# Juzhan/TAP-Net

Hardware: AMD Instinct MI355X
Metric: env-steps/s (batch placements) 2D n=10 LB_GREEDY; 1/2/4/8 GPU + CPU ref (higher is better)
Workload: dtype i32 height-maps / f64 candidate scores / f32 masks

## Files before the change

tap-net_amd/csrc/rolling.hip:

```cpp
#include <new>

#include "tap_common.h"
#include "tap_masks.h"
#include "tap_place.h"
#include "tap_waves.h"

struct RollArgs {
    int B, D, N, child, W, L, H, arm;
    const int32_t *blocks;
    const int32_t *positions;
    unsigned long long *rel;
    unsigned long long *state;
    const int64_t *remove_ptr;
    float *static_out;
    float *dynamic_out;
    float *colsum_out;
    unsigned long long *bits_out;
    float *cur_mask_out;
    int32_t *nodes_out;
    int32_t *err_out;
    int err_sticky;
    int wt;
};

__device__ __forceinline__ LaneRole roll_lane_role(int v, const float *dy, int C4, int RP, int rows)
{
#ifdef TAP_STREAM_UNALIGNED
    const int add = 0;
#else
    const int add = ((RP * C4) & 3) == 0 ? (int)((reinterpret_cast<uintptr_t>(dy) >> 4) & 3) : 0;
#endif
    return stream_lane_role(v, 0, C4, RP, 65536 / C4 + 1, 0, add, (rows + RP - 1) / RP);
}

__device__ __forceinline__ bool rng_meet(int a0, int a1, int b0, int b1) { return a0 < b1 && b0 < a1; }

template <int D>
__global__ void __launch_bounds__(TAP_BLOCK) k_rolling_init(RollArgs a)
{
    __shared__ int s_blk[TAP_BLOCK / 64][64 * 3];
    __shared__ int s_pos[TAP_BLOCK / 64][64 * 3];
    const int w = threadIdx.x >> 6, b = threadIdx.x & 63;
    const int inst = blockIdx.x * (TAP_BLOCK / 64) + w;
    const int n = a.N;
    if (inst < a.B)
        for (int k = b; k < n * D; k += 64) {
            s_blk[w][k] = a.blocks[(size_t)inst * n * D + k];
            s_pos[w][k] = a.positions[(size_t)inst * n * D + k];
        }
    tap_wave_lds_sync();
    if (inst >= a.B) return;
    if (b == 0) { a.state[(size_t)inst * 2] = 0; a.state[(size_t)inst * 2 + 1] = 0; }
    if (b >= n) return;
    const int *blk = s_blk[w], *pos = s_pos[w];
#define BX(i) blk[(i) * D]
#define BY(i) (D == 3 ? blk[(i) * D + 1] : 1)
// ... 348 lines not shown
                    if (dy) dy[(size_t)(sec * child + rm) * nRc + col] = (float)((m[sec] >> node) & 1ull);
            }
        }
    }
    
    if (!packed) return;
    tap_wave_lds_sync();
    PROF(6);
    const int C4 = nRc >> 2, RP = 64 / C4;
    if (dy && v < RP * C4) {
        const LaneRole role = roll_lane_role(v, dy, C4, RP, rows);
        const int c4 = role.c4;
        const u64 w0 = S.cw[c4 * 4], w1 = S.cw[c4 * 4 + 1], w2 = S.cw[c4 * 4 + 2], w3 = S.cw[c4 * 4 + 3];
        float4 *dst = reinterpret_cast<float4 *>(dy) + c4;
        int rw = role.r0;
        for (int i = 0; i < role.nq; ++i, rw += RP) {
            if ((unsigned)rw >= (unsigned)rows) continue;
            store_stream(&dst[(size_t)rw * C4], make_float4(bit_as_float(w0, rw), bit_as_float(w1, rw), bit_as_float(w2, rw),
                                                            bit_as_float(w3, rw)), a.wt);
        }
    }
    PROF(7);
}

template <int D, int CH>
__device__ __forceinline__ void rolling_emit_fast_tail(const RollArgs &a, int inst, int v, RollLds &S)
{
    constexpr int R = D == 2 ? 2 : 6, NRC = CH * R, C4 = NRC / 4, RP = 64 / C4, ROWS = 3 * CH, QN = (ROWS + RP - 1) / RP;
#if defined(TAP_PROF)
    long long tp = clock64();
#endif
    float *st = a.static_out + (size_t)inst * (1 + D) * NRC;
    float *dy = a.dynamic_out ? a.dynamic_out + (size_t)inst * ROWS * NRC : nullptr;
    if (v < NRC) {
        const int col = v, r = v / CH, cm = v - r * CH;
        const int pz = D == 3 ? (0x126 >> (2 * r)) & 3 : 1 - r;
        const bool guarded = pz == 0 || (D == 3 && pz == 1);
        const int k1 = pz == 0 ? 1 : 3;
        const unsigned ws0 = S.f.iw[cm];
        const unsigned r1 = S.f.iw[k1 * CH + cm], r2 = S.f.iw[(k1 + 1) * CH + cm];
        const unsigned ws1 = guarded ? r1 : 0u, ws2 = guarded ? r2 : 0u;
        const int c0 = __popc(ws0), c1 = __popc(ws1), c2 = __popc(ws2);
        if (a.colsum_out) {
            a.colsum_out[((size_t)inst * 3 + 0) * NRC + col] = (float)c0;
            a.colsum_out[((size_t)inst * 3 + 1) * NRC + col] = (float)c1;
            a.colsum_out[((size_t)inst * 3 + 2) * NRC + col] = (float)c2;
        }
        if (a.cur_mask_out) a.cur_mask_out[(size_t)inst * NRC + col] = (c1 * c2 + c0 != 0) ? 0.f : 1.f;
        const unsigned w = ws0 | (ws1 << CH) | (ws2 << (2 * CH));
        S.f.cw32[col] = w;
        if (a.bits_out) a.bits_out[(size_t)inst * NRC + col] = (u64)w;
        st[col] = (float)cm;
        const int r4 = 4 * r;
        const int o0 = D == 3 ? (0x884400 >> r4) & 15 : (0x40 >> r4) & 15;
        const int o1 = D == 3 ? (0x408084 >> r4) & 15 : (0x04 >> r4) & 15;
        const char *row = reinterpret_cast<const char *>(&S.f.dims[cm][0]);
        st[(size_t)1 * NRC + col] = (float)*reinterpret_cast<const int *>(row + o0);
        st[(size_t)2 * NRC + col] = (float)*reinterpret_cast<const int *>(row + o1);
        if (D == 3) {
            const int o2 = (0x040848 >> r4) & 15;
            st[(size_t)3 * NRC + col] = (float)*reinterpret_cast<const int *>(row + o2);
        }
    }
    tap_wave_lds_sync();
    PROF(6);
    {
        constexpr int K = RP * C4;
        constexpr bool AL = (K & 3) == 0;
#ifdef TAP_STREAM_UNALIGNED
        const int sb = 0;
#else
        const int sb = AL ? __builtin_amdgcn_readfirstlane((int)((reinterpret_cast<uintptr_t>(dy) >> 4) & 3)) : 0;
#endif
        if (dy && v < K) {
            int role = v - sb;
            const int late = role < 0 ? 1 : 0;
            role += late ? K : 0;
            const int rsub = role / C4, c4 = role - rsub * C4;
            const uint4 cq = *reinterpret_cast<const uint4 *>(&S.f.cw32[c4 * 4]);
            unsigned mk = 0u;
#pragma unroll
            for (int q = 0; q < QN; ++q) mk |= 1u << (RP * q);
            unsigned il = (cq.x >> rsub) & mk;
            il |= ((cq.y >> rsub) & mk) << 1;
            il |= ((cq.z >> rsub) & mk) << 2;
            il |= ((cq.w >> rsub) & mk) << 3;
            float4 *dst = reinterpret_cast<float4 *>(dy) + c4 + (size_t)rsub * C4;
            constexpr int NI = QN + ((AL && RP * (QN - 1) + (K - 3) / C4 < ROWS) ? 1 : 0);
            int q = -late;
#pragma unroll
            for (int i = 0; i < NI; ++i, ++q) {
                if (q >= 0 && RP * q + rsub < ROWS) {
                    const unsigned nib = (il >> (RP * q)) & 15u;
                    store_stream(&dst[(size_t)RP * q * C4], *reinterpret_cast<const float4 *>(&S.f.lut[nib][0]), a.wt);
                }
            }
        }
// ... 700 lines not shown
                               uint64_t *bits_out, float *current_mask_out, int32_t *nodes_out,
                               int32_t *err_out, void *stream, int err_sticky);

extern "C" int tap_rolling_window(tap_ctx *ctx, int B, int D, int N, int child, const int32_t *blocks,
                                  const uint64_t *rel, uint64_t *state, const int64_t *remove_ptr,
                                  float *static_out, float *dynamic_out, float *colsum_out,
                                  uint64_t *bits_out, float *current_mask_out, int32_t *nodes_out,
                                  int32_t *err_out, void *stream)
{
    return rolling_window_impl(ctx, B, D, N, child, blocks, rel, state, remove_ptr, static_out, dynamic_out, colsum_out,
                               bits_out, current_mask_out, nodes_out, err_out, stream, 0);
}

static int rolling_window_impl(tap_ctx *ctx, int B, int D, int N, int child, const int32_t *blocks,
                               const uint64_t *rel, uint64_t *state, const int64_t *remove_ptr,
                               float *static_out, float *dynamic_out, float *colsum_out,
                               uint64_t *bits_out, float *current_mask_out, int32_t *nodes_out,
                               int32_t *err_out, void *stream, int err_sticky)
{
    int rc = roll_check(ctx, B, D, N, child);
    if (rc) return rc;
    if (!blocks || !rel || !state || !static_out) return tap_fail(ctx, TAP_E_INVALID, "null pointer");
    if (!dynamic_out && !bits_out)
        return tap_fail(ctx, TAP_E_INVALID, "dynamic_out may only be left out when bits_out takes the window's bit shadow");
    RollArgs a = {};
    a.err_sticky = err_sticky;
    a.wt = tap_write_through((size_t)B * 3 * child * child * (D == 2 ? 2 : 6) * sizeof(float));
    a.B = B; a.D = D; a.N = N; a.child = child; a.blocks = blocks;
    a.rel = reinterpret_cast<unsigned long long *>(const_cast<uint64_t *>(rel));
    a.state = reinterpret_cast<unsigned long long *>(state);
    a.remove_ptr = remove_ptr; a.static_out = static_out; a.dynamic_out = dynamic_out;
    a.colsum_out = colsum_out; a.cur_mask_out = current_mask_out; a.nodes_out = nodes_out; a.err_out = err_out;
    a.bits_out = reinterpret_cast<unsigned long long *>(bits_out);
    if (bits_out && (3 * child > 64 || (child * (D == 2 ? 2 : 6)) % 4 != 0 || child * (D == 2 ? 2 : 6) > 256))
        return tap_fail(ctx, TAP_E_UNSUPPORTED, "bits_out needs 3*child <= 64, (child*R) %% 4 == 0, child*R <= 256");
    const int grid = (B + TAP_BLOCK / 64 - 1) / (TAP_BLOCK / 64);
    if (grid == 0) return TAP_OK;
    if (const int nw = roll_wide_nw(N, child)) {
        hipStream_t s_ = (hipStream_t)stream;
#define TAP_ROLL_WIDE(D_) do { \
            if (nw == 2) hipLaunchKernelGGL((k_rolling_window<D_, ROLL_CH_WIDE>), dim3(grid), dim3(TAP_BLOCK), 0, s_, ROLL_HOT_ARGS(a), a); \
            else if (nw == 3) hipLaunchKernelGGL((k_rolling_window_wide<D_, 3>), dim3(grid), dim3(TAP_BLOCK), 0, s_, ROLL_HOT_ARGS(a), a); \
            else hipLaunchKernelGGL((k_rolling_window_wide<D_, 4>), dim3(grid), dim3(TAP_BLOCK), 0, s_, ROLL_HOT_ARGS(a), a); } while (0)
        if (D == 2) TAP_ROLL_WIDE(2); else TAP_ROLL_WIDE(3);
#undef TAP_ROLL_WIDE
        TAP_LAUNCH_CHECK(ctx, "k_rolling_window(wide)");
        tap_variant_hit(ctx, TAP_HIT_ROLL_WINDOW, D, 0, nw == 2 ? TapVariant{0, ROLL_CH_WIDE, 0} : TapVariant{1, nw, 0}, a.wt);
        return TAP_OK;
    }
    if (N > 64) {
        const int g2 = (B + 63) / 64;
        hipStream_t s_ = (hipStream_t)stream;
#define TAP_ROLL_BIG(D_) do { \
            if (N <= 256) hipLaunchKernelGGL((k_rolling_window_big<D_, 4>), dim3(g2), dim3(64), 0, s_, a); \
            else if (N <= 1024) hipLaunchKernelGGL((k_rolling_window_big<D_, 16>), dim3(g2), dim3(64), 0, s_, a); \
            else hipLaunchKernelGGL((k_rolling_window_big<D_, 64>), dim3(g2), dim3(64), 0, s_, a); } while (0)
        if (D == 2) TAP_ROLL_BIG(2); else TAP_ROLL_BIG(3);
#undef TAP_ROLL_BIG
        TAP_LAUNCH_CHECK(ctx, "k_rolling_window_big");
        tap_variant_hit(ctx, TAP_HIT_ROLL_WINDOW, D, 0, TapVariant{2, 0, N <= 256 ? 4 : N <= 1024 ? 16 : 64}, a.wt);
        return TAP_OK;
    }
    const bool fast = roll_fast_ok(D, child);
    if (D == 2) {
        if (fast) hipLaunchKernelGGL((k_rolling_window<2, 10>), dim3(grid), dim3(TAP_BLOCK), 0, (hipStream_t)stream, ROLL_HOT_ARGS(a), a);
        else hipLaunchKernelGGL((k_rolling_window<2, 0>), dim3(grid), dim3(TAP_BLOCK), 0, (hipStream_t)stream, ROLL_HOT_ARGS(a), a);
// ... 44 lines not shown
{
    int rc = tap_desc_validate(ctx, d);
    if (rc) return rc;
    if (d->B == 0) return TAP_OK;
    rc = roll_check(ctx, d->B, d->D, N, child);
    if (rc) return rc;
    if (!env_state || !blocks || !rel || !state || !ptr || !static_cur || !static_next || static_cur == static_next)
        return tap_fail(ctx, TAP_E_INVALID, "bad rolling_step arguments (static_cur and static_next must differ)");
    if (!dynamic_out && !bits_out)
        return tap_fail(ctx, TAP_E_INVALID, "dynamic_out may only be left out when bits_out takes the window's bit shadow");
    if (d->strategy != TAP_LB_GREEDY || tap_is_big(d) || (N > 64 && roll_wide_nw(N, child) != 2)) {
        rc = tap_env_step_gather(ctx, d, env_state, static_cur, 1 + d->D, child * (d->D == 2 ? 2 : 6), ptr, nullptr,
                                 feature_out, stream);
        if (rc == TAP_OK && aux) {
            StepArgs s = {};
            s.d = *d; s.static_ = static_cur; s.static_rows = 1 + d->D; s.nR = child * (d->D == 2 ? 2 : 6); s.ptr = ptr;
            s.dec_static_out = aux->dec_static_out; s.tour_out = aux->tour_out; s.picked_out = aux->picked_out;
            s.nodes_cur = aux->nodes_cur; s.child = child; s.tour_stride = aux->tour_stride; s.tour_col = aux->tour_col;
            rc = tap_step_aux_launch(ctx, s, (hipStream_t)stream);
        }
        return rc ? rc : rolling_window_impl(ctx, d->B, d->D, N, child, blocks, rel, state, ptr, static_next, dynamic_out,
                                             colsum_out, bits_out, current_mask_out, nodes_out, err_out, stream, aux != nullptr);
    }
    RollStepArgs a = {};
    const int R = d->D == 2 ? 2 : 6;
    a.r.err_sticky = aux != nullptr;
    a.r.wt = tap_write_through((size_t)d->B * 3 * child * child * R * sizeof(float));
    a.r.B = d->B; a.r.D = d->D; a.r.N = N; a.r.child = child; a.r.blocks = blocks;
    a.r.rel = reinterpret_cast<unsigned long long *>(const_cast<uint64_t *>(rel));
    a.r.state = reinterpret_cast<unsigned long long *>(state);
    a.r.remove_ptr = ptr; a.r.static_out = static_next; a.r.dynamic_out = dynamic_out;
    a.r.colsum_out = colsum_out; a.r.cur_mask_out = current_mask_out; a.r.nodes_out = nodes_out; a.r.err_out = err_out;
    a.r.bits_out = reinterpret_cast<unsigned long long *>(bits_out);
    if (bits_out && (3 * child > 64 || (child * R) % 4 != 0 || child * R > 256))
        return tap_fail(ctx, TAP_E_UNSUPPORTED, "bits_out needs 3*child <= 64, (child*R) %% 4 == 0, child*R <= 256");
    a.s.d = *d;
    tap_env_layout(d, env_state, &a.s.v);
    a.s.static_ = static_cur; a.s.static_rows = 1 + d->D; a.s.nR = child * R; a.s.ptr = ptr;
    a.s.feature_out = feature_out; a.s.flen = tap_env_feature_len(d);
    a.s.lut = ctx ? ctx->stab_lut : nullptr;
    if (aux) {
        a.s.dec_static_out = aux->dec_static_out; a.s.tour_out = aux->tour_out; a.s.picked_out = aux->picked_out;
        a.s.nodes_cur = aux->nodes_cur; a.s.child = child; a.s.tour_stride = aux->tour_stride; a.s.tour_col = aux->tour_col;
    }
    const int Gs = tap_group_size(d);
    hipStream_t st = (hipStream_t)stream;
    if (d->D == 2) {
        if (Gs == 8) return launch_rolling_step<2, 8>(ctx, a, st);
        if (Gs == 16) return launch_rolling_step<2, 16>(ctx, a, st);
        if (Gs == 32) return launch_rolling_step<2, 32>(ctx, a, st);
        return launch_rolling_step<2, 64>(ctx, a, st);
    }
    if (Gs == 8) return launch_rolling_step<3, 8>(ctx, a, st);
    if (Gs == 16) return launch_rolling_step<3, 16>(ctx, a, st);
    if (Gs == 32) return launch_rolling_step<3, 32>(ctx, a, st);
    return launch_rolling_step<3, 64>(ctx, a, st);
}

extern "C" int tap_rolling_step(tap_ctx *ctx, const tap_env_desc *d, void *env_state, int N, int child,
                                const int32_t *blocks, const uint64_t *rel, uint64_t *state,
                                const int64_t *ptr, const float *static_cur, float *static_next,
                                float *dynamic_out, float *colsum_out, uint64_t *bits_out,
                                float *current_mask_out, int32_t *nodes_out, int32_t *err_out,
                                float *feature_out, void *stream)
{
    return rolling_step_impl(ctx, d, env_state, N, child, blocks, rel, state, ptr, static_cur, static_next, dynamic_out,
// ... 93 lines not shown
```

tap-net_amd/csrc/tap_masks.h:

```cpp
#pragma once

#include <hip/hip_runtime.h>

#include <cstdint>
#include <type_traits>
#include <cstdlib>

#include "tap_stream_variant.h"

constexpr size_t TAP_WT_MAX_BYTES = 64u << 20;

struct MaskArgs {
    int B, n, R, nR, rows, update_rows, static_rows;
    const float *dyn_in;
    float *dyn_out;
    const float *static_;
    const int64_t *ptr;
    const float *mask_in;
    const float *cs_in;
    float *cs_out;
    float *cur_out;
    float *mask_out;
    const unsigned long long *bits_in;
    unsigned long long *bits_out;
    int *nonbinary;
    int c4_magic, rp;
    int wt;
    int sb_mul, sb_add, nq, nq2;
    int inplace;
};

inline int tap_write_through(size_t bytes);

constexpr int TAP_HOT_MAGIC_MASK = 0xffffff, TAP_HOT_SB_MUL_SHIFT = 24, TAP_HOT_SB_ADD_SHIFT = 26, TAP_HOT_SB_MASK = 3;

inline MaskArgs mask_finish(MaskArgs a)
{
    const int c4 = a.nR >> 2;
    a.c4_magic = c4 > 0 ? 65536 / c4 + 1 : 0;
    static_assert(65536 + 1 <= TAP_HOT_MAGIC_MASK, "c4_magic shares its kernel argument with sb_mul / sb_add (TAP_MASK_HOT_ARGS)");
    a.rp = c4 > 0 ? 64 / c4 : 0;
    a.wt = tap_write_through((size_t)a.B * a.rows * a.nR * sizeof(float));
    const bool al = a.wt && c4 > 0 && ((a.rp * c4) & 3) == 0;
    a.sb_mul = al ? (a.rows * c4) & 3 : 0;
    a.sb_add = al ? (int)((reinterpret_cast<uintptr_t>(a.dyn_out) >> 4) & 3) : 0;
    a.nq = a.rp > 0 ? (a.rows + a.rp - 1) / a.rp : 0;
    a.nq2 = a.rp > 0 ? (2 * a.rows + a.rp - 1) / a.rp : 0;
    return a;
}

struct LaneRole {
    int rsub, c4;
    int r0;
    int nq;
    int sb;
};

__device__ __forceinline__ LaneRole stream_lane_role(int lane, int env, int C4, int RP, int c4_magic, int sb_mul, int sb_add, int nq)
{
    const int sb = __builtin_amdgcn_readfirstlane((env * sb_mul + sb_add) & 3);
    int role = lane - sb;
    const bool late = role < 0;
    role += late ? RP * C4 : 0;
    LaneRole o;
    o.rsub = (int)(((unsigned)role * (unsigned)c4_magic) >> 16);
    o.c4 = role - o.rsub * C4;
    o.r0 = o.rsub - (late ? RP : 0);
    o.nq = nq + (sb != 0);
    o.sb = sb;
    return o;
}

__host__ __device__ __forceinline__ bool mask_builds_bits(const MaskArgs &a) { return !a.bits_in && a.bits_out && a.dyn_in; }

#define TAP_MASK_HOT_PARAMS const int64_t *h_ptr, const float *h_static, const float *h_mask_in, const void *h_src, int h_B, \
                            int h_nR, int h_static_rows, int h_c4_magic
#define TAP_MASK_HOT_NAMES h_ptr, h_static, h_mask_in, h_src, h_B, h_nR, h_static_rows, h_c4_magic
#define TAP_MASK_HOT_ARGS(m) (m).ptr, (m).static_, (m).mask_in,                                                              \
        ((m).bits_in ? static_cast<const void *>((m).bits_in) : static_cast<const void *>((m).dyn_in)), (m).B, (m).nR,       \
        (m).static_rows, ((m).c4_magic | (((m).sb_mul & TAP_HOT_SB_MASK) << TAP_HOT_SB_MUL_SHIFT) |                           \
                          (((m).sb_add & TAP_HOT_SB_MASK) << TAP_HOT_SB_ADD_SHIFT))
__device__ __forceinline__ MaskArgs tap_mask_hot(const MaskArgs &k, bool src_is_bits, TAP_MASK_HOT_PARAMS)
{
    MaskArgs m = k;
    m.ptr = h_ptr; m.static_ = h_static; m.mask_in = h_mask_in;
    m.B = h_B; m.nR = h_nR; m.static_rows = h_static_rows; m.c4_magic = h_c4_magic & TAP_HOT_MAGIC_MASK;
    m.sb_mul = (h_c4_magic >> TAP_HOT_SB_MUL_SHIFT) & TAP_HOT_SB_MASK; m.sb_add = (h_c4_magic >> TAP_HOT_SB_ADD_SHIFT) & TAP_HOT_SB_MASK;
    if (src_is_bits) m.bits_in = static_cast<const unsigned long long *>(h_src);
    else m.dyn_in = static_cast<const float *>(h_src);
    return m;
}


#ifdef TAP_PROF
constexpr int TAP_PROF_WGS = 2048, TAP_PROF_WAVES = 16;
static __device__ unsigned long long tap_prof_tl[TAP_PROF_WGS * TAP_PROF_WAVES * 4];
#define TL_STAMP(i) do { if ((threadIdx.x & 63) == 0 && blockIdx.x < TAP_PROF_WGS) \
        tap_prof_tl[(blockIdx.x * TAP_PROF_WAVES + (threadIdx.x >> 6)) * 4 + (i)] = __builtin_amdgcn_s_memrealtime(); } while (0)
#define TL_WAIT_VM() __builtin_amdgcn_s_waitcnt(0)
#else
#define TL_STAMP(i) do { } while (0)
#define TL_WAIT_VM() do { } while (0)
#endif

__device__ __forceinline__ void tap_wave_lds_sync_m()
{
    __builtin_amdgcn_fence(__ATOMIC_RELEASE, "wavefront");
    __builtin_amdgcn_wave_barrier();
    __builtin_amdgcn_fence(__ATOMIC_ACQUIRE, "wavefront");
}

__device__ __forceinline__ void store_stream(float4 *dst, const float4 &v, int wt)
{
    typedef float v4f __attribute__((ext_vector_type(4)));
    const v4f nv = {v.x, v.y, v.z, v.w};
    if (wt) asm volatile("global_store_dwordx4 %0, %1, off sc0 sc1\n\ts_nop 1" : : "v"(dst), "v"(nv) : "memory");
    else __builtin_nontemporal_store(nv, reinterpret_cast<v4f *>(dst));
}

inline int tap_write_through(size_t bytes, size_t limit)
{
    static const int forced = [] { const char *e = getenv("TAP_WRITE_THROUGH"); return e ? (e[0] != '0') : -1; }();
    if (forced >= 0) return forced;
    return bytes <= limit;
}
inline int tap_write_through(size_t bytes) { return tap_write_through(bytes, TAP_WT_MAX_BYTES); }

__device__ __forceinline__ float bit_as_float(unsigned long long w, int r)
{
    const unsigned half = r < 32 ? (unsigned)w : (unsigned)(w >> 32);
    return (float)((half >> (r & 31)) & 1u);
}

__device__ __forceinline__ long tap_mod_col(long p, int n, int nR)
{
    if ((unsigned long)p >= (unsigned long)nR) p = 0;
    while (p >= n) p -= n;
    return p;
}

__device__ __forceinline__ void mask_column(const MaskArgs &a, int env, int j, long real_m,
                                            float move, float small, float large)
{
    float keep = a.mask_in ? a.mask_in[(size_t)env * a.nR + j] : 1.f;
    if (a.ptr)
        for (int r = 0; r < a.R; ++r)
            if (j == real_m + (long)a.n * r) keep = 0.f;
    if (a.mask_out) a.mask_out[(size_t)env * a.nR + j] = keep;
// ... 200 lines not shown
    for (int r = 0; r < 5; ++r) v = v >= n ? v - n : v;
    while (v >= n) v -= n;
    return v;
}

template <int NS, int NC, bool BUILD = false, bool MERGED = true, int C4S = 0, bool INPLACE = false, bool FULL = false>
__device__ __forceinline__ void stream_wave_bits_r4(const MaskArgs &a, int senv0, int lane, const bool (&on_)[NS],
                                                 float *lds = nullptr)
{
    static_assert(!(BUILD && INPLACE), "the first step on a fresh tensor writes all of it");
    bool on[NS];
#pragma unroll
    for (int k = 0; k < NS; ++k) on[k] = FULL ? true : on_[k];
#if defined(TAP_STREAM_LOAD_BJ)
    constexpr bool BJ_X = false;
#elif defined(TAP_STREAM_BJX_ALL)
    constexpr bool BJ_X = !BUILD && NC == 1 && (C4S == 5 || C4S == 15);
#else
    constexpr bool BJ_X = !BUILD && NC == 1 && NS == 1 && (C4S == 5 || C4S == 15);
#endif
    typedef unsigned long long u64;
    static_assert(NS <= 2, "a stream wave expands one or two slabs");
    if (!on[0]) return;
    const int nR = C4S ? 4 * C4S : a.nR, C4 = C4S ? C4S : nR >> 2, rows = C4S ? (C4S == 10 ? 60 : 30) : a.rows, n = C4S ? (C4S == 10 ? 20 : 10) : a.n;
    const int RP = C4S ? 64 / C4S : a.rp;
    const int c4_magic = C4S ? 65536 / C4S + 1 : a.c4_magic;
    const bool lane_on = lane < RP * C4;
#ifdef TAP_STREAM_UNALIGNED
    const LaneRole role = stream_lane_role(lane, 0, C4, RP, c4_magic, 0, 0, 0);
#else
    const LaneRole role = stream_lane_role(lane, senv0, C4, RP, c4_magic, a.sb_mul, a.sb_add, 0);
#endif
    const bool first_row = role.rsub == 0;
    u64 *tile = reinterpret_cast<u64 *>(lds);
    const void *any = BUILD ? static_cast<const void *>(a.dyn_in) : static_cast<const void *>(a.bits_in);
    const bool has_ptr = FULL || a.ptr != nullptr, has_static = FULL || a.static_ != nullptr, has_mask = FULL || a.mask_in != nullptr;
    const int64_t *ptrp = has_ptr ? a.ptr : static_cast<const int64_t *>(any);
    const float *stp = has_static ? a.static_ : static_cast<const float *>(any);
    const float *mip = has_mask ? a.mask_in : static_cast<const float *>(any);
    long praw[NS];
    float row0[NS][NC], keep[NS][NC];
    u64 bj[NS][NC];
    ulonglong2 w[NS][2];
#pragma unroll
    for (int k = 0; k < NS; ++k) {
        const int env = on[k] ? senv0 + k : senv0;
        praw[k] = ptrp[has_ptr ? env : 0];
        const float *strow = stp + (has_static ? (size_t)env * a.static_rows * nR : (size_t)0);
        const float *mirow = mip + (has_mask ? (size_t)env * nR : (size_t)0);
#pragma unroll
        for (int c = 0; c < NC; ++c) {
            const unsigned j = (unsigned)min(lane + 64 * c, nR - 1);
            row0[k][c] = strow[has_static ? j : 0u];
            keep[k][c] = mirow[has_mask ? j : 0u];
        }
    }
#ifdef TAP_STREAM_G2
    __builtin_amdgcn_s_waitcnt(0x0F70);
#endif
    if (!BUILD) {
#pragma unroll
        for (int k = 0; k < NS; ++k) {
            const int env = on[k] ? senv0 + k : senv0;
            const unsigned long long *brow = a.bits_in + (size_t)env * nR;
            if constexpr (!BJ_X) {
#pragma unroll
                for (int c = 0; c < NC; ++c) bj[k][c] = brow[(unsigned)min(lane + 64 * c, nR - 1)];
            }
            const ulonglong2 *src = reinterpret_cast<const ulonglong2 *>(brow) + (unsigned)(role.c4 * 2);
            w[k][0] = src[0];
            w[k][1] = src[1];
        }
    }
    if (BUILD) {
        stream_build_bits<NS>(a, senv0, lane, on, tile);
#pragma unroll
        for (int k = 0; k < NS; ++k) {
#pragma unroll
            for (int c = 0; c < NC; ++c) bj[k][c] = tile[(size_t)k * nR + min(lane + 64 * c, nR - 1)];
            const ulonglong2 *src = reinterpret_cast<const ulonglong2 *>(tile + (size_t)k * nR + role.c4 * 4);
            w[k][0] = src[0];
            w[k][1] = src[1];
        }
    }
    float *o_dyn = a.dyn_out, *o_cur = a.cur_out, *o_mask = a.mask_out;
    unsigned long long *o_bits = a.bits_out;
    int o_wt = a.wt;
#ifdef TAP_STREAM_EARLY_ARGS
    asm volatile("" : "+s"(o_dyn), "+s"(o_cur), "+s"(o_mask), "+s"(o_bits), "+s"(o_wt));
#endif
    __builtin_amdgcn_s_waitcnt(0x0F70);
#ifdef TAP_PROF
    TL_STAMP(1);
#endif
    const u64 nmask = (n >= 64) ? ~0ull : ((1ull << n) - 1ull);
    auto mod_n = [&](int v) -> int {
        if constexpr (C4S != 0) return (int)((unsigned)v % (unsigned)(C4S == 10 ? 20 : 10));
        else return tap_mod_small(v, n);
    };
    int jm[NC];
#pragma unroll
    for (int c = 0; c < NC; ++c) jm[c] = mod_n(min(lane + 64 * c, nR - 1));
    u64 clr[NS];
    int pm[NS], realk[NS];
    constexpr int UR_C = C4S != 0 ? 3 : 0;
    const int ur = UR_C ? UR_C : a.update_rows;
#pragma unroll
    for (int k = 0; k < NS; ++k) {
        const bool valid_v = on[k] && has_ptr && praw[k] >= 0 && praw[k] < nR;
#ifdef TAP_STREAM_VPICK
        constexpr bool SPICK = false;
#else
        constexpr bool SPICK = NS > 1;
#endif
        bool valid;
        int p, real;
        if constexpr (!SPICK) {
            valid = valid_v;
            p = valid ? (int)praw[k] : 0;
            float r0 = -1.f;
// ... 105 lines not shown
                                                 (float)((m2 >> r) & 1u), (float)((m3 >> r) & 1u));
                    store_stream(&dst[(size_t)rr * C4], v, o_wt);
                }
#else
                if (o_wt) run(std::integral_constant<int, 1>{}); else run(std::integral_constant<int, 0>{});
#endif
            } else if (rows <= 32) {
                for (int i = 0; i < nq; ++i, rr += RP) {
                    if ((unsigned)rr >= (unsigned)total) continue;
                    const bool up = NS > 1 && rr >= rows;
                    const int r = up ? rr - rows : rr;
                    const unsigned m0 = up ? (unsigned)nw[NS - 1][0] : (unsigned)nw[0][0], m1 = up ? (unsigned)nw[NS - 1][1] : (unsigned)nw[0][1],
                                   m2 = up ? (unsigned)nw[NS - 1][2] : (unsigned)nw[0][2], m3 = up ? (unsigned)nw[NS - 1][3] : (unsigned)nw[0][3];
                    const float4 v = make_float4((float)((m0 >> r) & 1u), (float)((m1 >> r) & 1u),
                                                 (float)((m2 >> r) & 1u), (float)((m3 >> r) & 1u));
                    store_stream(&dst[(size_t)rr * C4], v, o_wt);
                }
            } else {
                for (int i = 0; i < nq; ++i, rr += RP) {
                    if ((unsigned)rr >= (unsigned)total) continue;
                    const bool up = NS > 1 && rr >= rows;
                    const int r = up ? rr - rows : rr;
                    const float4 v = make_float4(bit_as_float(up ? nw[NS - 1][0] : nw[0][0], r), bit_as_float(up ? nw[NS - 1][1] : nw[0][1], r),
                                                 bit_as_float(up ? nw[NS - 1][2] : nw[0][2], r), bit_as_float(up ? nw[NS - 1][3] : nw[0][3], r));
                    store_stream(&dst[(size_t)rr * C4], v, o_wt);
                }
            }
        }
        if (first_row && o_bits) {
#pragma unroll
            for (int k = 0; k < NS; ++k) {
                if (!on[k]) continue;
                ulonglong2 *dst = reinterpret_cast<ulonglong2 *>(o_bits + (size_t)(senv0 + k) * nR + role.c4 * 4);
                dst[0] = make_ulonglong2(nw[k][0], nw[k][1]);
                dst[1] = make_ulonglong2(nw[k][2], nw[k][3]);
            }
        }
    }
    unsigned nbx[NS];
    if constexpr (BJ_X) {
        const int jj = min(lane, nR - 1);
        const int src = ((jj >> 2) + role.sb) << 2;
        const int e = jj & 3;
#pragma unroll
        for (int k = 0; k < NS; ++k) {
            const int e0 = __builtin_amdgcn_ds_bpermute(src, (int)(unsigned)nw[k][0]), e1 = __builtin_amdgcn_ds_bpermute(src, (int)(unsigned)nw[k][1]);
            const int e2 = __builtin_amdgcn_ds_bpermute(src, (int)(unsigned)nw[k][2]), e3 = __builtin_amdgcn_ds_bpermute(src, (int)(unsigned)nw[k][3]);
            nbx[k] = (unsigned)(e == 0 ? e0 : e == 1 ? e1 : e == 2 ? e2 : e3);
        }
    }
#pragma unroll
    for (int k = 0; k < NS; ++k) {
        if (!on[k]) continue;
        const int env = senv0 + k;
#pragma unroll
        for (int c = 0; c < NC; ++c) {
            const int j = lane + 64 * c;
            if (j >= nR) continue;
            const u64 nb = BJ_X ? (u64)nbx[k] : (bj[k][c] & ~clr[k]);
            const int move = __popcll(nb & nmask), small = n >= 64 ? 0 : __popcll((nb >> n) & nmask);
            const int large = n >= 32 ? 0 : __popcll((nb >> (2 * n)) & nmask);
            const float kp = (jm[c] == pm[k]) ? 0.f : (has_mask ? keep[k][c] : 1.f);
            if (o_mask) o_mask[(size_t)env * nR + j] = kp;
            if (o_cur) o_cur[(size_t)env * nR + j] = (small * large + move) != 0 ? 0.f : kp;
        }
    }
}

#ifdef TAP_STREAM_R3
template <int NS, int NC, bool BUILD = false>
__device__ __forceinline__ void stream_wave_bits_r3(const MaskArgs &a, int senv0, int lane, const bool (&on)[NS],
// ... 282 lines not shown
```

tap-net_amd/csrc/transition_macs.hip:

```cpp
#include <cstdlib>

#include "tap_common.h"
#include "tap_macs.h"
#include "tap_macs3.h"
#include "tap_masks.h"
#include "tap_place.h"
#include "tap_transition.h"
#include "tap_waves.h"

#ifndef TAP_MACS_SW
#define TAP_MACS_SW 4
#endif
template <int G, int NC, int MODE, int WC = 0>
__global__ void __launch_bounds__((TransGeom<G, TAP_MACS_SW>::THREADS)) k_transition_macs(TransArgs a)
{
    using Geo = TransGeom<G, TAP_MACS_SW>;
    constexpr int EPB = Geo::EPB, SPW = Geo::SPW, ENV_WAVES = Geo::ENV_WAVES;
    extern __shared__ float trans_lds[];
    const int tid = threadIdx.x, wave = tid >> 6, lane = tid & 63;
    const int env_base = blockIdx.x * EPB;
    const int B = a.s.d.B, W = WC ? WC : a.s.d.W, H = a.s.d.H;
    if (wave >= ENV_WAVES) {
        trans_stream_wave<SPW, NC, MODE>(a.m, env_base + (wave - ENV_WAVES) * SPW, lane,
                                     trans_lds + (size_t)(wave - ENV_WAVES) * SPW * 3 * a.m.nR);
// ... 123 lines not shown
    const TapVariant v = tap_stream_variant(TAP_SV_MACS3, tap_mask_facts(a.m), TapLaunchFacts{3, G, EPB, a.s.d.B, a.s.d.W, a.s.d.L, false});
    return tap_launch_variant<TAP_SV_MACS3, 3, G>(ctx, "k_transition_macs3", v, a.m.wt, [&](auto k) -> int {
        using K = decltype(k);
        TAP_HIP_CHECK(ctx, tap_allow_lds(k_transition_macs3<G, K::nc, K::mode, K::extra>, lds));
        hipLaunchKernelGGL((k_transition_macs3<G, K::nc, K::mode, K::extra>), dim3(grid), dim3(THREADS), lds, st, a);
        return TAP_OK;
    });
}

int tap_macs_validate(tap_ctx *ctx, const tap_env_desc &d);

template <int G> static int launch_transition_macs(tap_ctx *ctx, const TransArgs &a, hipStream_t st)
{
    constexpr int EPB = TransGeom<G, TAP_MACS_SW>::EPB, THREADS = TransGeom<G, TAP_MACS_SW>::THREADS;
    const int grid = (a.s.d.B + EPB - 1) / EPB;
    if (grid == 0) return TAP_OK;
    const size_t lds = (size_t)EPB * 3 * a.m.nR * sizeof(float) +
                       (size_t)EPB * macs_group_words(G, a.s.d.H, a.s.d.n_max, a.s.d.W) * sizeof(int);
    if (lds > tap_lds_limit(ctx)) return tap_fail(ctx, TAP_E_UNSUPPORTED, "transition(MACS): %zu bytes of LDS needed", lds);
    const TapVariant v = tap_stream_variant(TAP_SV_MACS, tap_mask_facts(a.m), TapLaunchFacts{2, G, EPB, a.s.d.B, a.s.d.W, a.s.d.L, false});
    return tap_launch_variant<TAP_SV_MACS, 2, G>(ctx, "k_transition_macs", v, a.m.wt, [&](auto k) -> int {
        using K = decltype(k);
        TAP_HIP_CHECK(ctx, tap_allow_lds(k_transition_macs<G, K::nc, K::mode, K::extra>, lds));
        hipLaunchKernelGGL((k_transition_macs<G, K::nc, K::mode, K::extra>), dim3(grid), dim3(THREADS), lds, st, a);
        return TAP_OK;
    });
}


int tap_transition_macs_launch(tap_ctx *ctx, const tap_env_desc *d, const TransArgs &a0, hipStream_t st)
{
    TransArgs a = a0;
    a.m.wt = tap_write_through((size_t)a.m.B * a.m.rows * a.m.nR * sizeof(float), (size_t)128 << 20);
    const int Gs = tap_group_size(d);
    if (d->D == 3) {
        switch (Gs) {
        case 8: return launch_transition_macs3<8>(ctx, a, st);
        case 16: return launch_transition_macs3<16>(ctx, a, st);
        case 32: return launch_transition_macs3<32>(ctx, a, st);
        default: return launch_transition_macs3<64>(ctx, a, st);
        }
    }
    return d->W <= 8 ? launch_transition_macs<8>(ctx, a, st) : launch_transition_macs<16>(ctx, a, st);
}
```

Baseline: 1.483 billion.

## Emit mask, bits and static tails as 16-byte quad write-through stores

```diff
diff --git a/tap-net_amd/csrc/rolling.hip b/tap-net_amd/csrc/rolling.hip
--- a/tap-net_amd/csrc/rolling.hip
+++ b/tap-net_amd/csrc/rolling.hip
@@ -21,7 +21,18 @@
     int32_t *err_out;
     int err_sticky;
     int wt;
+    int wtq;
 };
+
+static inline int roll_quad_tail(const RollArgs &a)
+{
+#ifdef TAP_NO_ROLL_QUAD
+    return 0;
+#else
+    const uintptr_t al = reinterpret_cast<uintptr_t>(a.static_out) | reinterpret_cast<uintptr_t>(a.cur_mask_out) | reinterpret_cast<uintptr_t>(a.bits_out);
+    return a.wt && al % 16 == 0;
+#endif
+}
 
 __device__ __forceinline__ LaneRole roll_lane_role(int v, const float *dy, int C4, int RP, int rows)
 {
@@ -436,6 +447,8 @@
 #endif
     float *st = a.static_out + (size_t)inst * (1 + D) * NRC;
     float *dy = a.dynamic_out ? a.dynamic_out + (size_t)inst * ROWS * NRC : nullptr;
+    const bool qt = a.wtq != 0;
+    static_assert(RP >= 1 + D, "the quad tail: one row group per row of static");
     if (v < NRC) {
         const int col = v, r = v / CH, cm = v - r * CH;
         const int pz = D == 3 ? (0x126 >> (2 * r)) & 3 : 1 - r;
@@ -450,23 +463,59 @@
             a.colsum_out[((size_t)inst * 3 + 1) * NRC + col] = (float)c1;
             a.colsum_out[((size_t)inst * 3 + 2) * NRC + col] = (float)c2;
         }
-        if (a.cur_mask_out) a.cur_mask_out[(size_t)inst * NRC + col] = (c1 * c2 + c0 != 0) ? 0.f : 1.f;
+        if (!qt && a.cur_mask_out) a.cur_mask_out[(size_t)inst * NRC + col] = (c1 * c2 + c0 != 0) ? 0.f : 1.f;
         const unsigned w = ws0 | (ws1 << CH) | (ws2 << (2 * CH));
         S.f.cw32[col] = w;
-        if (a.bits_out) a.bits_out[(size_t)inst * NRC + col] = (u64)w;
-        st[col] = (float)cm;
-        const int r4 = 4 * r;
-        const int o0 = D == 3 ? (0x884400 >> r4) & 15 : (0x40 >> r4) & 15;
-        const int o1 = D == 3 ? (0x408084 >> r4) & 15 : (0x04 >> r4) & 15;
-        const char *row = reinterpret_cast<const char *>(&S.f.dims[cm][0]);
-        st[(size_t)1 * NRC + col] = (float)*reinterpret_cast<const int *>(row + o0);
-        st[(size_t)2 * NRC + col] = (float)*reinterpret_cast<const int *>(row + o1);
-        if (D == 3) {
-            const int o2 = (0x040848 >> r4) & 15;
-            st[(size_t)3 * NRC + col] = (float)*reinterpret_cast<const int *>(row + o2);
+        if (!qt && a.bits_out) a.bits_out[(size_t)inst * NRC + col] = (u64)w;
+        if (!qt) {
+            st[col] = (float)cm;
+            const int r4 = 4 * r;
+            const int o0 = D == 3 ? (0x884400 >> r4) & 15 : (0x40 >> r4) & 15;
+            const int o1 = D == 3 ? (0x408084 >> r4) & 15 : (0x04 >> r4) & 15;
+            const char *row = reinterpret_cast<const char *>(&S.f.dims[cm][0]);
+            st[(size_t)1 * NRC + col] = (float)*reinterpret_cast<const int *>(row + o0);
+            st[(size_t)2 * NRC + col] = (float)*reinterpret_cast<const int *>(row + o1);
+            if (D == 3) {
+                const int o2 = (0x040848 >> r4) & 15;
+                st[(size_t)3 * NRC + col] = (float)*reinterpret_cast<const int *>(row + o2);
+            }
         }
     }
     tap_wave_lds_sync();
+    if (qt && v < RP * C4) {
+        const int g = v / C4, c4 = v - g * C4;
+        const uint4 cq = *reinterpret_cast<const uint4 *>(&S.f.cw32[c4 * 4]);
+        const unsigned wq[4] = {cq.x, cq.y, cq.z, cq.w};
+        if (g <= D) {
+            float sv[4];
+#pragma unroll
+            for (int i = 0; i < 4; ++i) {
+                const int col = c4 * 4 + i, r = col / CH, cm = col - r * CH, r4 = 4 * r;
+                const int o0 = D == 3 ? (0x884400 >> r4) & 15 : (0x40 >> r4) & 15;
+                const int o1 = D == 3 ? (0x408084 >> r4) & 15 : (0x04 >> r4) & 15;
+                const int o2 = D == 3 ? (0x040848 >> r4) & 15 : 0;
+                const int o = g == 1 ? o0 : g == 2 ? o1 : o2;
+                const char *row = reinterpret_cast<const char *>(&S.f.dims[cm][0]);
+                sv[i] = g == 0 ? (float)cm : (float)*reinterpret_cast<const int *>(row + o);
+            }
+            store_stream(reinterpret_cast<float4 *>(st + (size_t)g * NRC + c4 * 4), make_float4(sv[0], sv[1], sv[2], sv[3]), 1);
+        }
+        if (g == 0) {
+            constexpr unsigned F0 = (1u << CH) - 1u;
+            if (a.cur_mask_out) {
+                float cm4[4];
+#pragma unroll
+                for (int i = 0; i < 4; ++i)
+                    cm4[i] = ((wq[i] & F0) != 0 || ((wq[i] & (F0 << CH)) != 0 && (wq[i] & (F0 << (2 * CH))) != 0)) ? 0.f : 1.f;
+                store_stream(reinterpret_cast<float4 *>(a.cur_mask_out + (size_t)inst * NRC + c4 * 4), make_float4(cm4[0], cm4[1], cm4[2], cm4[3]), 1);
+            }
+            if (a.bits_out) {
+                ulonglong2 *bd = reinterpret_cast<ulonglong2 *>(a.bits_out + (size_t)inst * NRC + c4 * 4);
+                store_stream(&bd[0], make_ulonglong2((u64)wq[0], (u64)wq[1]), 1);
+                store_stream(&bd[1], make_ulonglong2((u64)wq[2], (u64)wq[3]), 1);
+            }
+        }
+    }
     PROF(6);
     {
         constexpr int K = RP * C4;
@@ -1233,6 +1282,7 @@
     a.remove_ptr = remove_ptr; a.static_out = static_out; a.dynamic_out = dynamic_out;
     a.colsum_out = colsum_out; a.cur_mask_out = current_mask_out; a.nodes_out = nodes_out; a.err_out = err_out;
     a.bits_out = reinterpret_cast<unsigned long long *>(bits_out);
+    a.wtq = roll_quad_tail(a);
     if (bits_out && (3 * child > 64 || (child * (D == 2 ? 2 : 6)) % 4 != 0 || child * (D == 2 ? 2 : 6) > 256))
         return tap_fail(ctx, TAP_E_UNSUPPORTED, "bits_out needs 3*child <= 64, (child*R) %% 4 == 0, child*R <= 256");
     const int grid = (B + TAP_BLOCK / 64 - 1) / (TAP_BLOCK / 64);
@@ -1343,6 +1393,7 @@
     a.r.remove_ptr = ptr; a.r.static_out = static_next; a.r.dynamic_out = dynamic_out;
     a.r.colsum_out = colsum_out; a.r.cur_mask_out = current_mask_out; a.r.nodes_out = nodes_out; a.r.err_out = err_out;
     a.r.bits_out = reinterpret_cast<unsigned long long *>(bits_out);
+    a.r.wtq = roll_quad_tail(a.r);
     if (bits_out && (3 * child > 64 || (child * R) % 4 != 0 || child * R > 256))
         return tap_fail(ctx, TAP_E_UNSUPPORTED, "bits_out needs 3*child <= 64, (child*R) %% 4 == 0, child*R <= 256");
     a.s.d = *d;
diff --git a/tap-net_amd/csrc/tap_masks.h b/tap-net_amd/csrc/tap_masks.h
--- a/tap-net_amd/csrc/tap_masks.h
+++ b/tap-net_amd/csrc/tap_masks.h
@@ -26,6 +26,7 @@
     int *nonbinary;
     int c4_magic, rp;
     int wt;
+    int wtq;
     int sb_mul, sb_add, nq, nq2;
     int inplace;
 };
@@ -33,14 +34,27 @@
 inline int tap_write_through(size_t bytes);
 
 constexpr int TAP_HOT_MAGIC_MASK = 0xffffff, TAP_HOT_SB_MUL_SHIFT = 24, TAP_HOT_SB_ADD_SHIFT = 26, TAP_HOT_SB_MASK = 3;
-
-inline MaskArgs mask_finish(MaskArgs a)
+constexpr int TAP_HOT_WTQ_SHIFT = 28;
+
+static inline int mask_quad_tail(const MaskArgs &a)
+{
+#ifdef TAP_NO_QUAD_TAIL
+    return 0;
+#else
+    const bool shape = a.update_rows == 3 && ((a.n == 10 && a.rows == 30 && (a.nR == 20 || a.nR == 60)) || (a.n == 20 && a.rows == 60 && a.nR == 40));
+    const uintptr_t al = reinterpret_cast<uintptr_t>(a.mask_in) | reinterpret_cast<uintptr_t>(a.mask_out) | reinterpret_cast<uintptr_t>(a.cur_out);
+    return a.wt && shape && al % 16 == 0;
+#endif
+}
+
+static inline MaskArgs mask_finish(MaskArgs a)
 {
     const int c4 = a.nR >> 2;
     a.c4_magic = c4 > 0 ? 65536 / c4 + 1 : 0;
     static_assert(65536 + 1 <= TAP_HOT_MAGIC_MASK, "c4_magic shares its kernel argument with sb_mul / sb_add (TAP_MASK_HOT_ARGS)");
     a.rp = c4 > 0 ? 64 / c4 : 0;
     a.wt = tap_write_through((size_t)a.B * a.rows * a.nR * sizeof(float));
+    a.wtq = mask_quad_tail(a);
     const bool al = a.wt && c4 > 0 && ((a.rp * c4) & 3) == 0;
     a.sb_mul = al ? (a.rows * c4) & 3 : 0;
     a.sb_add = al ? (int)((reinterpret_cast<uintptr_t>(a.dyn_out) >> 4) & 3) : 0;
@@ -79,13 +93,14 @@
 #define TAP_MASK_HOT_ARGS(m) (m).ptr, (m).static_, (m).mask_in,                                                              \
         ((m).bits_in ? static_cast<const void *>((m).bits_in) : static_cast<const void *>((m).dyn_in)), (m).B, (m).nR,       \
         (m).static_rows, ((m).c4_magic | (((m).sb_mul & TAP_HOT_SB_MASK) << TAP_HOT_SB_MUL_SHIFT) |                           \
-                          (((m).sb_add & TAP_HOT_SB_MASK) << TAP_HOT_SB_ADD_SHIFT))
+                          (((m).sb_add & TAP_HOT_SB_MASK) << TAP_HOT_SB_ADD_SHIFT) | (((m).wtq & 1) << TAP_HOT_WTQ_SHIFT))
 __device__ __forceinline__ MaskArgs tap_mask_hot(const MaskArgs &k, bool src_is_bits, TAP_MASK_HOT_PARAMS)
 {
     MaskArgs m = k;
     m.ptr = h_ptr; m.static_ = h_static; m.mask_in = h_mask_in;
     m.B = h_B; m.nR = h_nR; m.static_rows = h_static_rows; m.c4_magic = h_c4_magic & TAP_HOT_MAGIC_MASK;
     m.sb_mul = (h_c4_magic >> TAP_HOT_SB_MUL_SHIFT) & TAP_HOT_SB_MASK; m.sb_add = (h_c4_magic >> TAP_HOT_SB_ADD_SHIFT) & TAP_HOT_SB_MASK;
+    m.wtq = (h_c4_magic >> TAP_HOT_WTQ_SHIFT) & 1;
     if (src_is_bits) m.bits_in = static_cast<const unsigned long long *>(h_src);
     else m.dyn_in = static_cast<const float *>(h_src);
     return m;
@@ -110,10 +125,13 @@
     __builtin_amdgcn_fence(__ATOMIC_ACQUIRE, "wavefront");
 }
 
-__device__ __forceinline__ void store_stream(float4 *dst, const float4 &v, int wt)
-{
+template <class T>
+__device__ __forceinline__ void store_stream(T *dst, const T &v, int wt)
+{
+    static_assert(sizeof(T) == 16 && alignof(T) == 16, "a 16-byte store");
     typedef float v4f __attribute__((ext_vector_type(4)));
-    const v4f nv = {v.x, v.y, v.z, v.w};
+    v4f nv;
+    __builtin_memcpy(&nv, &v, 16);
     if (wt) asm volatile("global_store_dwordx4 %0, %1, off sc0 sc1\n\ts_nop 1" : : "v"(dst), "v"(nv) : "memory");
     else __builtin_nontemporal_store(nv, reinterpret_cast<v4f *>(dst));
 }
@@ -380,6 +398,7 @@
     const LaneRole role = stream_lane_role(lane, senv0, C4, RP, c4_magic, a.sb_mul, a.sb_add, 0);
 #endif
     const bool first_row = role.rsub == 0;
+    const bool qt = C4S != 0 && a.wtq;
     u64 *tile = reinterpret_cast<u64 *>(lds);
     const void *any = BUILD ? static_cast<const void *>(a.dyn_in) : static_cast<const void *>(a.bits_in);
     const bool has_ptr = FULL || a.ptr != nullptr, has_static = FULL || a.static_ != nullptr, has_mask = FULL || a.mask_in != nullptr;
@@ -387,8 +406,9 @@
     const float *stp = has_static ? a.static_ : static_cast<const float *>(any);
     const float *mip = has_mask ? a.mask_in : static_cast<const float *>(any);
     long praw[NS];
-    float row0[NS][NC], keep[NS][NC];
-    u64 bj[NS][NC];
+    float row0[NS][NC], keep[NS][NC] = {};
+    float4 keep4[NS] = {};
+    u64 bj[NS][NC] = {};
     ulonglong2 w[NS][2];
 #pragma unroll
     for (int k = 0; k < NS; ++k) {
@@ -400,8 +420,9 @@
         for (int c = 0; c < NC; ++c) {
             const unsigned j = (unsigned)min(lane + 64 * c, nR - 1);
             row0[k][c] = strow[has_static ? j : 0u];
-            keep[k][c] = mirow[has_mask ? j : 0u];
-        }
+            if (!qt) keep[k][c] = mirow[has_mask ? j : 0u];
+        }
+        if (qt) keep4[k] = reinterpret_cast<const float4 *>(mirow)[has_mask ? (unsigned)role.c4 : 0u];
     }
 #ifdef TAP_STREAM_G2
     __builtin_amdgcn_s_waitcnt(0x0F70);
@@ -412,8 +433,10 @@
             const int env = on[k] ? senv0 + k : senv0;
             const unsigned long long *brow = a.bits_in + (size_t)env * nR;
             if constexpr (!BJ_X) {
-#pragma unroll
-                for (int c = 0; c < NC; ++c) bj[k][c] = brow[(unsigned)min(lane + 64 * c, nR - 1)];
+                if (!qt) {
+#pragma unroll
+                    for (int c = 0; c < NC; ++c) bj[k][c] = brow[(unsigned)min(lane + 64 * c, nR - 1)];
+                }
             }
             const ulonglong2 *src = reinterpret_cast<const ulonglong2 *>(brow) + (unsigned)(role.c4 * 2);
             w[k][0] = src[0];
@@ -424,8 +447,10 @@
         stream_build_bits<NS>(a, senv0, lane, on, tile);
 #pragma unroll
         for (int k = 0; k < NS; ++k) {
-#pragma unroll
-            for (int c = 0; c < NC; ++c) bj[k][c] = tile[(size_t)k * nR + min(lane + 64 * c, nR - 1)];
+            if (!qt) {
+#pragma unroll
+                for (int c = 0; c < NC; ++c) bj[k][c] = tile[(size_t)k * nR + min(lane + 64 * c, nR - 1)];
+            }
             const ulonglong2 *src = reinterpret_cast<const ulonglong2 *>(tile + (size_t)k * nR + role.c4 * 4);
             w[k][0] = src[0];
             w[k][1] = src[1];
@@ -434,6 +459,10 @@
     float *o_dyn = a.dyn_out, *o_cur = a.cur_out, *o_mask = a.mask_out;
     unsigned long long *o_bits = a.bits_out;
     int o_wt = a.wt;
+#ifdef TAP_SMALL_NOSTORE
+    o_cur = o_mask = nullptr;
+    o_bits = nullptr;
+#endif
 #ifdef TAP_STREAM_EARLY_ARGS
     asm volatile("" : "+s"(o_dyn), "+s"(o_cur), "+s"(o_mask), "+s"(o_bits), "+s"(o_wt));
 #endif
@@ -605,11 +634,51 @@
             for (int k = 0; k < NS; ++k) {
                 if (!on[k]) continue;
                 ulonglong2 *dst = reinterpret_cast<ulonglong2 *>(o_bits + (size_t)(senv0 + k) * nR + role.c4 * 4);
-                dst[0] = make_ulonglong2(nw[k][0], nw[k][1]);
-                dst[1] = make_ulonglong2(nw[k][2], nw[k][3]);
-            }
-        }
-    }
+#ifdef TAP_BITS_WT
+                const bool through = o_wt != 0;
+#else
+                const bool through = qt;
+#endif
+                if (through) {
+                    store_stream(&dst[0], make_ulonglong2(nw[k][0], nw[k][1]), 1);
+                    store_stream(&dst[1], make_ulonglong2(nw[k][2], nw[k][3]), 1);
+                } else {
+                    dst[0] = make_ulonglong2(nw[k][0], nw[k][1]);
+                    dst[1] = make_ulonglong2(nw[k][2], nw[k][3]);
+                }
+            }
+        }
+        if constexpr (C4S != 0) {
+            if (qt && first_row) {
+                constexpr int N_C = C4S == 10 ? 20 : 10;
+                constexpr u64 F0 = (1ull << N_C) - 1ull, F1 = F0 << N_C, F2 = F0 << (2 * N_C);
+                const int j0 = role.c4 * 4;
+#pragma unroll
+                for (int k = 0; k < NS; ++k) {
+                    if (!on[k]) continue;
+                    const float kin[4] = {keep4[k].x, keep4[k].y, keep4[k].z, keep4[k].w};
+                    float km[4], kc[4];
+#pragma unroll
+                    for (int q = 0; q < 4; ++q) {
+                        km[q] = (mod_n(j0 + q) == pm[k]) ? 0.f : (has_mask ? kin[q] : 1.f);
+                        bool busy;
+                        if constexpr (C4S == 10) {
+                            const u64 nb = nw[k][q];
+                            busy = (nb & F0) != 0 || ((nb & F1) != 0 && (nb & F2) != 0);
+                        } else {
+                            const unsigned nb = (unsigned)nw[k][q];
+                            busy = (nb & (unsigned)F0) != 0 || ((nb & (unsigned)F1) != 0 && (nb & (unsigned)F2) != 0);
+                        }
+                        kc[q] = busy ? 0.f : km[q];
+                    }
+                    const size_t o = (size_t)(senv0 + k) * nR + j0;
+                    if (o_mask) store_stream(reinterpret_cast<float4 *>(o_mask + o), make_float4(km[0], km[1], km[2], km[3]), 1);
+                    if (o_cur) store_stream(reinterpret_cast<float4 *>(o_cur + o), make_float4(kc[0], kc[1], kc[2], kc[3]), 1);
+                }
+            }
+        }
+    }
+    if (qt) return;
     unsigned nbx[NS];
     if constexpr (BJ_X) {
         const int jj = min(lane, nR - 1);
diff --git a/tap-net_amd/csrc/transition_macs.hip b/tap-net_amd/csrc/transition_macs.hip
--- a/tap-net_amd/csrc/transition_macs.hip
+++ b/tap-net_amd/csrc/transition_macs.hip
@@ -179,6 +179,7 @@
 {
     TransArgs a = a0;
     a.m.wt = tap_write_through((size_t)a.m.B * a.m.rows * a.m.nR * sizeof(float), (size_t)128 << 20);
+    a.m.wtq = mask_quad_tail(a.m);
     const int Gs = tap_group_size(d);
     if (d->D == 3) {
         switch (Gs) {
```

Result: slower. 1.215 billion (-18.1%).
